# Ipsedo/MARLClassification

Measured on AMD Instinct MI355X. Metric: agent-env-steps/sec, higher is better.
Workload: dtype f32; 1 GPU; RESISC45 256x256x3, 16 agents, 16 steps, f=12, README dims (configs[2]); full train iteration: rollout + A2C loss + BPTT backward + Adam; batch_per_gpu=256, global_batch=256, parallelism=dp1, rng=library (Philox4x32-10), launch=eager

## Files before the change

marlclassification_amd/csrc/episode.hip:

```cpp
#include <math.h>
#include <stdlib.h>
#include <string.h>

#include "../../include/marl_hip_rowops.h"
#include "../../include/marl_hip_cnnops.h"
#include "../../include/marl_hip_explore.h"
#include "../../include/marl_hip_classloss.h"
#include "../../include/marl_hip_softtargets.h"
#include "common.h"

namespace marl {

struct Dims {
    int na, nb, ns;
    int64_t R, NR;
    int H, W, c_img, f;
    int L;
    int ch[MARL_MAX_CNN_LAYERS + 1];
    int grp[MARL_MAX_CNN_LAYERS];
    int hw[MARL_MAX_CNN_LAYERS + 1];
    int P[MARL_MAX_CNN_LAYERS];
    int K[MARL_MAX_CNN_LAYERS];
    int ldk[MARL_MAX_CNN_LAYERS];
    int nf, nin;
// ... 1503 lines not shown
                    MARL_P_PRE_LNW, MARL_P_PRE_LNB, NR, d.nlb, grads, 0));
    MARL_TRY(tn(c, c.at(c.e.DAQ1), d.ld_nlb, c.Hs(1), d.ld_nb, MARL_P_PRE_W0, d.nlb, d.n_b, NR, grads[MARL_P_PRE_B0]));
    MARL_TRY(tn(c, c.at(c.e.DVAL), 4, c.at(c.e.AC1), d.ld_nla, MARL_P_CRI_W1, 1, d.nla, NR, grads[MARL_P_CRI_B1]));
    if (d.nla <= 384) {
        MARL_TRY(ln_bwd_rank(c, c.at(c.e.DVAL), 4, 1, MARL_P_CRI_W1, c.at(c.e.ZC1), d.ld_nla,
                             c.at(c.e.STC1), MARL_P_CRI_LNW, MARL_P_CRI_LNB, NR, d.nla, grads,
                             c.at(c.e.DAC1), d.ld_nla));
    } else {
        MARL_TRY(gemm1(c, gemm_prob(c.at(c.e.DVAL), 4, c.wtB(MARL_P_CRI_W1), c.at(c.e.DAC1),
                                    d.ld_nla, (int)NR, d.nla)));
        MARL_TRY(ln_bwd(c, c.at(c.e.DAC1), d.ld_nla, c.at(c.e.ZC1), d.ld_nla, c.at(c.e.STC1),
                        MARL_P_CRI_LNW, MARL_P_CRI_LNB, NR, d.nla, grads, 0));
    }
    MARL_TRY(tn(c, c.at(c.e.DAC1), d.ld_nla, c.HCs(1), d.ld_na, MARL_P_CRI_W0, d.nla, d.n_a, NR, grads[MARL_P_CRI_B0]));
    if (sb && sb->g_probs) g_probs = sb->g_probs;
    const Explore& ex = c.opt.explore;
    if (ex.on && (ex.inv_tau != 1.f || ex.eps != 0.f))
        MARL_TRY(launch_policy_dlogits_explore(g_logp, g_probs, c.PROBSs(0), c.ACTs(0), c.at(c.e.DLOG), d.ld_nA, NR,
                                               d.nA, ex.inv_tau, ex.keep, ex.eps / (float)d.nA, st));
    else if (g_probs)
        MARL_TRY(launch_policy_dlogits_probs(g_logp, g_probs, c.PROBSs(0), c.ACTs(0), c.at(c.e.DLOG),
                                             d.ld_nA, NR, d.nA, st));
    else
        MARL_TRY(launch_policy_dlogits(g_logp, c.PROBSs(0), c.ACTs(0), c.at(c.e.DLOG), d.ld_nA, NR,
                                       d.nA, st));
    MARL_TRY(tn(c, c.at(c.e.DLOG), d.ld_nA, c.at(c.e.AP1, 0), d.ld_nla, MARL_P_POL_W1, d.nA, d.nla, NR, grads[MARL_P_POL_B1]));
    if (d.nA <= 4 && d.nla <= 384) {
        MARL_TRY(ln_bwd_rank(c, c.at(c.e.DLOG), d.ld_nA, d.nA, MARL_P_POL_W1, c.at(c.e.ZP1, 0),
                             d.ld_nla, c.at(c.e.STP1, 0), MARL_P_POL_LNW, MARL_P_POL_LNB, NR, d.nla,
                             grads, c.at(c.e.DAP1), d.ld_nla));
    } else {
        MARL_TRY(gemm1(c, gemm_prob(c.at(c.e.DLOG), d.ld_nA, c.wtB(MARL_P_POL_W1),
                                    c.at(c.e.DAP1), d.ld_nla, (int)NR, d.nla)));
        MARL_TRY(ln_bwd(c, c.at(c.e.DAP1), d.ld_nla, c.at(c.e.ZP1, 0), d.ld_nla, c.at(c.e.STP1, 0),
                        MARL_P_POL_LNW, MARL_P_POL_LNB, NR, d.nla, grads, 0));
    }
    MARL_TRY(tn(c, c.at(c.e.DAP1), d.ld_nla, c.HCs(1), d.ld_na, MARL_P_POL_W0, d.nla, d.n_a, NR, grads[MARL_P_POL_B0]));
    {
        GemmProb ph = gemm_prob(c.at(c.e.DAQ1), d.ld_nlb, c.wtB(MARL_P_PRE_W0), c.DHs(1), d.ld_nb, (int)NR, d.n_b);
        GemmProb pa = gemm_prob(c.at(c.e.DAP1), d.ld_nla, c.wtB(MARL_P_POL_W0), c.DHCs(1), d.ld_na, (int)NR, d.n_a);
        gemm_add_seg(pa, c.at(c.e.DAC1), d.ld_nla, c.wtB(MARL_P_CRI_W0));
        MARL_TRY(gemm2(c, ph, pa));
    }
    if (sb) {
        MARL_TRY(launch_acc2d(c.DHs(ns), d.ld_nb, sb->g_h, d.n_b, d.R, d.n_b, st));
        MARL_TRY(launch_acc2d(c.DHCs(ns), d.ld_na, sb->g_hc, d.n_a, d.R, d.n_a, st));
    }

    s.heads_early = c.opt.heads_event != nullptr && !sb;
    if (s.heads_early) {
        if (c.tq) MARL_TRY(launch_tn_queue(s.tq, c.rq, st));
        MARL_TRY(s.rq.flush());
        MARL_TRY(unpack_grads(c, grads, 1));
        MARL_HIP_CHECK(hipEventRecord(c.opt.heads_event, st));
    }
    return MARL_OK;
}


static int enc_bwd_rows(const BwdState& s, int t, int acc, float* dh) {
    const Ctx& c = s.c;
    const Dims& d = c.d;
    const int R = (int)d.R;
    float* dze2 = c.at(c.e.DZE2) + (size_t)t * d.R * d.ld_nm;
    float* dae1 = c.at(c.e.DAE1) + (size_t)t * d.R * d.ld_nm2;
    MARL_TRY(ln_bwd(c, dze2, d.ld_nm, c.at(c.e.ZE2, t), d.ld_nm, c.at(c.e.STE2, t), MARL_P_ENC_LN1W,
                    MARL_P_ENC_LN1B, d.R, d.n_m, s.grads, acc));
    MARL_TRY(gemm1(c, gemm_prob(dze2, d.ld_nm, c.wtB(MARL_P_ENC_W1), dae1, d.ld_nm2, R, d.nm2)));
    MARL_TRY(ln_bwd(c, dae1, d.ld_nm2, c.at(c.e.ZE1, t), d.ld_nm2, c.at(c.e.STE1, t), MARL_P_ENC_LN0W,
                    MARL_P_ENC_LN0B, d.R, d.nm2, s.grads, acc));
    return gemm1(c, gemm_prob(dae1, d.ld_nm2, c.wtB(MARL_P_ENC_W0), dh, d.ld_nb, R, d.n_b, nullptr, 1));
}

static int bwd_recurrent(const BwdState& s, int t, float* ddbar, float* ddbar2) {
    const Ctx& c = s.c;
    const Dims& d = c.d;
    const int R = (int)d.R;
    const struct { int which, w, row0; float* out; int ldo, n, acc; } prod[4] = {
        {0, MARL_P_LB_WHH, 0, c.DHs(t), d.ld_nb, d.n_b, 1},
        {1, MARL_P_LA_WHH, 0, c.DHCs(t), d.ld_na, d.n_a, 1},
        {0, MARL_P_LB_WIH, d.nf, ddbar, d.ld_dbl, d.n_mo + d.n_d, 0},
        {1, MARL_P_LA_WIH, d.nf, ddbar2, d.ld_dbl, d.n_mo + d.n_d, 0}};
    const int count = c.plan.panels_bwd ? 4 : 2;
    if (c.plan.panels_bwd && c.e.g3) {
        G3Batch g{};
        for (int i = 0; i < count; ++i) {
            const auto& q = prod[i];
            g.p[i] = g3_prob(c.img(q.which ? c.e.GA3 : c.e.GB3), (int)((int64_t)t * d.R), c.wt3k(q.w), q.row0,
                             4 * (q.which ? d.n_a : d.n_b), q.out, q.ldo, R, q.n, nullptr, q.acc);
        }
        g.count = count;
        return launch_gemm_nt3(g, c.st);
    }
    GemmBatch gb{};
    for (int i = 0; i < count; ++i) {
        const auto& q = prod[i];
        gb.p[i] = gemm_prob(c.at(q.which ? c.e.GA : c.e.GB, t), q.which ? d.ld_ga : d.ld_gb,
                            c.wtB(q.w).from_row(q.row0), q.out, q.ldo, R, q.n, nullptr, q.acc);
    }
    gb.count = count;
    if (!c.plan.panels_bwd) {
        GemmProb& p = gb.p[gb.count++];
        p = gemm_prob(c.at(c.e.GB, t), d.ld_gb, c.wtB(MARL_P_LB_WIH).from_row(d.nf), ddbar, d.ld_dbl, R, d.n_mo);
        gemm_add_seg(p, c.at(c.e.GA, t), d.ld_ga, c.wtB(MARL_P_LA_WIH).from_row(d.nf));
    }
    return launch_gemm_nt(gb, c.st);
}

static void fill_dec_bwd_prob(BwdState& s, int t, float* ddbar, float* ddbar2, PanelBwdProb& pd) {
    const Ctx& c = s.c;
    const Dims& d = c.d;
    pd.da = ddbar;
    pd.ldda = d.ld_dbl;
    pd.da2 = ddbar2;
    pd.ldda2 = d.ld_dbl;
    pd.m = (int)d.R;
    pd.nlayers = 2;
    fill_dec_bwd_layers(c, t, (size_t)s.pln_blocks * 2, ddbar, c.at(c.e.DAD1) + (size_t)t * d.R * d.ld_nm2, pd.layer);
    pd.dx = c.at(c.e.DMBAR);
    pd.lddx = d.ld_nm;
    pd.accumulate = 0;
    if (t > 0) {
        pd.has_cell = 1;
        pd.cell = cell_bwd_args(c, 1, t - 1);
        pd.cell_rows = d.R;
        s.action_done = true;
    }
}

static int bwd_step_chain(BwdState& s, int t, float* ddbar, float* ddbar2) {
    const Ctx& c = s.c;
    const Dims& d = c.d;
    PanelBwdProb pd{};
    fill_dec_bwd_prob(s, t, ddbar, ddbar2, pd);
    pd.by_batch = panel_chain_by_batch(d.na);
    pd.g_na = d.na;
    pd.g_nb = d.nb;
    if (t > 0) {
        pd.nlayers = 4;
        pd.agg_at = 2;
        pd.mix = c.opt.comm;
        if (c.opt.comm) pd.gate = comm_gate(c, t);
        fill_enc_bwd_layers(c, t - 1, (size_t)s.pln_blocks * 2, pd.layer + 2);
        pd.dx = c.DHs(t);
        pd.lddx = d.ld_nb;
        pd.accumulate = 1;
        pd.has_cellb = 1;
        pd.cellb = cell_bwd_args(c, 0, t - 1);
        s.belief_done = true;
    }
    MARL_TRY(launch_panel_bwd(pd, c.st));
    return gate_image_fallback(c, pd, t - 1);
}

static int bwd_step_panels(BwdState& s, int t, float* ddbar, float* ddbar2) {
    const Ctx& c = s.c;
    const Dims& d = c.d;
    PanelBwdProb pd{};
    fill_dec_bwd_prob(s, t, ddbar, ddbar2, pd);
    MARL_TRY(launch_panel_bwd(pd, c.st));
    MARL_TRY(gate_image_fallback(c, pd, t - 1));
    if (t == 0) return MARL_OK;
    PanelBwdProb pe{};
    pe.da = c.at(c.e.DMBAR);
    pe.ldda = d.ld_nm;
    pe.agg_na = d.na;
    pe.agg_nb = d.nb;
    if (c.opt.comm) {
        MARL_TRY(mix_msg(c, t, c.at(c.e.DMBAR), c.at(c.e.DMBAR), d.ld_nm, 1));
        pe.agg_na = pe.agg_nb = 0;
    }
    pe.m = (int)d.R;
    pe.nlayers = 2;
    fill_enc_bwd_layers(c, t - 1, (size_t)s.pln_blocks * 2, pe.layer);
    pe.dx = c.DHs(t);
    pe.lddx = d.ld_nb;
    pe.accumulate = 1;
    return launch_panel_bwd(pe, c.st);
}

static int bwd_step_rows(const BwdState& s, int t, float* ddbar) {
    const Ctx& c = s.c;
    const Dims& d = c.d;
// ... 1472 lines not shown
```

marlclassification_amd/csrc/panel.hip:

```cpp
#include <stdlib.h>

#include "common.h"
#include "sample.h"

namespace marl {

typedef float f32x4 __attribute__((ext_vector_type(4)));

__device__ __forceinline__ void lds_barrier() {
    asm volatile("s_waitcnt lgkmcnt(0)\n\ts_barrier" ::: "memory");
}
__device__ __forceinline__ float mul_rn(float a, float b) {
#pragma clang fp contract(off)
    return a * b;
}
__device__ __forceinline__ float silu_p(float y) { return silu_fast(y); }
__device__ __forceinline__ float silu_grad_p(float y) { return silu_grad_fast(y); }

constexpr int kPanelRows = 16;
constexpr int kPanelMaxWaves = 12;
constexpr int kPanelMaxCols = 6;

__host__ __device__ inline int panel_stride(int k) { return ((k + 15) & ~15) + 4; }

// ... 66 lines not shown
    return ks < 1 ? 1 : ks;
}

constexpr int panel_kper_c(int K16, int ks) { return (((K16 + ks - 1) / ks) + 15) & ~15; }
constexpr int panel_ksplit_c(int K, int nt, int nwaves) {
    const int K16 = (K + 15) & ~15, want = (K16 + 63) / 64;
    int ks = nwaves / nt;
    ks = ks < want ? ks : want;
    return ks < 1 ? 1 : ks;
}
constexpr int panel_stride_c(int k) { return ((k + 15) & ~15) + 4; }
constexpr int cmax(int a, int b) { return a > b ? a : b; }

struct PanelDyn {
    static constexpr bool kStatic = false, kByBatch = false;
    static constexpr int kLayers = kPanelMaxLayers, kSoft = 0, kWaves = 0, kK0 = 0, kAggAt = 0, kKLast = 0;
    static constexpr int off_e = 0, off_prm = 0, off_colp = 0, off_part = 0, off_rowmap = 0;
    static constexpr int n(int) { return 0; }
    static constexpr int k(int) { return 0; }
};
template <int WAVES, int K0, int AGG_AT, int SOFT, int... N>
struct PanelNet {
    static constexpr bool kStatic = true, kByBatch = AGG_AT > 0;
    static constexpr int kLayers = (int)sizeof...(N), kSoft = SOFT, kWaves = WAVES, kK0 = K0, kAggAt = AGG_AT;
    static constexpr int n(int l) {
        constexpr int w[] = {N...};
        return w[l];
    }
    static constexpr int k(int l) { return l == 0 ? K0 : n(l - 1); }
    static constexpr int s0(int layers) {
        int v = kPanelRows * panel_stride_c(K0);
        for (int l = 1; l < layers; l += 2) v = cmax(v, kPanelRows * panel_stride_c(n(l)));
        return v;
    }
    static constexpr int s1(int layers) {
        int v = 0;
        for (int l = 0; l < layers; l += 2) v = cmax(v, kPanelRows * panel_stride_c(n(l)));
        return v;
    }
    static constexpr bool ok() {
        for (int l = 0; l < kLayers; ++l) {
            const int nt = (n(l) + 31) >> 5, K16 = (k(l) + 15) & ~15, ks = panel_ksplit_c(k(l), nt, WAVES);
            if (nt * ks > WAVES || (ks - 1) * panel_kper_c(K16, ks) >= K16) return false;
            if ((n(l) & 15) || (k(l) & 15) || n(l) > 64 * kPanelMaxCols) return false;
        }
        return WAVES >= 4 && WAVES <= kPanelMaxWaves && (SOFT == 0 || (s0(SOFT) == s0(kLayers) && s1(SOFT) == s1(kLayers)));
    }
};
template <int WAVES, int AGG_AT, int KLAST, int... N>
struct PanelBwdNet {
    static constexpr bool kStatic = true, kByBatch = true;
    static constexpr int kLayers = (int)sizeof...(N), kSoft = 0, kWaves = WAVES, kAggAt = AGG_AT, kKLast = KLAST;
    static constexpr int n(int l) {
        constexpr int w[] = {N...};
        return w[l];
    }
    static constexpr int k(int l) { return l + 1 < kLayers ? n(l + 1) : KLAST; }
    static constexpr int nmax() {
        int v = 0;
        for (int l = 0; l < kLayers; ++l) v = cmax(v, n(l));
        return v;
    }
    static constexpr int pmax() {
        int v = 0;
        for (int l = 0; l < kLayers; ++l) v = cmax(v, cmax(panel_stride_c(n(l)), panel_stride_c(k(l))));
        return v;
    }
    static constexpr int prm() {
        int v = 0;
        for (int l = 0; l < kLayers; ++l) v += 2 * n(l);
        return v;
    }
    static constexpr int off_e = kPanelRows * pmax(), off_prm = 2 * kPanelRows * pmax(), off_colp = off_prm + prm() + 16;
    static constexpr int off_part = off_colp + WAVES * 2 * nmax(), off_rowmap = off_part + (WAVES - 1) * 512;
    static constexpr bool ok() {
        for (int l = 0; l < kLayers; ++l) {
            const int nt = (k(l) + 31) >> 5, n16 = (n(l) + 15) & ~15, ks = panel_ksplit_c(n(l), nt, WAVES);
            if (nt > WAVES || (ks - 1) * panel_kper_c(n16, ks) >= n16) return false;
            if ((n(l) & 15) || (k(l) & 15)) return false;
        }
        return WAVES >= 8 && WAVES <= kPanelMaxWaves && nmax() <= 128 && (KLAST & 3) == 0;
    }
};

template <int K16, int KS, int KPER>
__device__ __forceinline__ void panel_gemm_st(f32x4 (&acc)[2], const float* in, int stride,
                                              const float* __restrict__ wfrag, int j, int s, int lane) {
    constexpr int groups = K16 >> 4, last0 = (KS - 1) * KPER;
    static_assert(last0 < K16 && (KPER & 15) == 0, "slice plan");
    const int quad = lane >> 4, l16 = lane & 15;
    const int kbeg = __builtin_amdgcn_readfirstlane(s * KPER);
    const float* arow = in + l16 * stride + 4 * quad + kbeg;
    const int g0 = __builtin_amdgcn_readfirstlane(j * groups + (kbeg >> 4));
    const float* wb = wfrag + (size_t)g0 * 512;
    const unsigned lo = 4u * (unsigned)lane;
#pragma unroll
    for (int r = 0; r < 4; ++r) acc[0][r] = acc[1][r] = 0.f;
#pragma unroll
    for (int c = 0; c < (KPER + 63) / 64; ++c) {
        if (last0 + 64 * c < K16 || kbeg + 64 * c < K16) {
            float4 b0[4], b1[4];
#pragma unroll
            for (int i = 0; i < 4; ++i) {
                if (64 * c + 16 * i < KPER) {
                    b0[i] = *reinterpret_cast<const float4*>(wb + 2048 * c + 512 * i + lo);
                    b1[i] = *reinterpret_cast<const float4*>(wb + 2048 * c + 512 * i + 256 + lo);
                }
            }
#pragma unroll
            for (int i = 0; i < 4; ++i) {
                if (64 * c + 16 * i < KPER && (last0 + 64 * c + 16 * i < K16 || kbeg + 64 * c + 16 * i < K16)) {
                    const float4 a = *reinterpret_cast<const float4*>(arow + 64 * c + 16 * i);
                    acc[0] = __builtin_amdgcn_mfma_f32_16x16x4f32(a.x, b0[i].x, acc[0], 0, 0, 0);
                    acc[1] = __builtin_amdgcn_mfma_f32_16x16x4f32(a.x, b1[i].x, acc[1], 0, 0, 0);
                    acc[0] = __builtin_amdgcn_mfma_f32_16x16x4f32(a.y, b0[i].y, acc[0], 0, 0, 0);
                    acc[1] = __builtin_amdgcn_mfma_f32_16x16x4f32(a.y, b1[i].y, acc[1], 0, 0, 0);
                    acc[0] = __builtin_amdgcn_mfma_f32_16x16x4f32(a.z, b0[i].z, acc[0], 0, 0, 0);
                    acc[1] = __builtin_amdgcn_mfma_f32_16x16x4f32(a.z, b1[i].z, acc[1], 0, 0, 0);
                    acc[0] = __builtin_amdgcn_mfma_f32_16x16x4f32(a.w, b0[i].w, acc[0], 0, 0, 0);
                    acc[1] = __builtin_amdgcn_mfma_f32_16x16x4f32(a.w, b1[i].w, acc[1], 0, 0, 0);
                }
            }
        }
    }
}

template <class SH, bool BWD, int L = 0>
__device__ __forceinline__ void panel_gemm_layer(int l, f32x4 (&acc)[2], const float* in, int stride,
                                                 const float* __restrict__ wfrag, int j, int s, int lane) {
    if constexpr (SH::kStatic && L < SH::kLayers) {
        if (l == L) {
            constexpr int K = BWD ? SH::n(L) : SH::k(L), nout = BWD ? SH::k(L) : SH::n(L);
            constexpr int K16 = (K + 15) & ~15, ks = panel_ksplit_c(K, (nout + 31) >> 5, SH::kWaves);
            panel_gemm_st<K16, ks, panel_kper_c(K16, ks)>(acc, in, stride, wfrag, j, s, lane);
        } else {
            panel_gemm_layer<SH, BWD, L + 1>(l, acc, in, stride, wfrag, j, s, lane);
        }
    }
}

template <int NC>
__device__ __forceinline__ void panel_ln_rows(const PanelLayer& Lr, float* outp, int ys, int n, const float* lgamma,
                                              const float* lbeta, const int* rowmap, int wave, int nwaves, int lane)
{
    constexpr int RPW = 4;
    float g[NC], bt[NC];
#pragma unroll
    for (int u = 0; u < NC; ++u) {
        const int c = lane + 64 * u;
        g[u] = c < n ? lgamma[c] : 0.f;
        bt[u] = c < n ? lbeta[c] : 0.f;
    }
    const float inv_n = 1.0f / (float)n;
#pragma unroll
    for (int i = 0; i < RPW; ++i) {
        const int lr = wave + i * nwaves;
        if (lr < kPanelRows) {
            float* zr = outp + lr * ys;
            const int row = rowmap[lr];
            float v[NC];
            float sm = 0.f;
#pragma unroll
            for (int u = 0; u < NC; ++u) {
                const int c = lane + 64 * u;
                v[u] = c < n ? zr[c] : 0.f;
                sm += v[u];
// ... 726 lines not shown
    {
        float pv[kPanelMaxLayers][2];
#pragma unroll
        for (int l = 0; l < kPanelMaxLayers; ++l) {
            pv[l][0] = pv[l][1] = 0.f;
            if (ST && l >= SH::kLayers) continue;
            if (l < nlayers && tid < (ST ? SH::n(l) : P.layer[l].n)) {
                pv[l][0] = P.layer[l].gamma[tid];
                pv[l][1] = P.layer[l].beta[tid];
            }
        }
        float cmv = 0.f;
        if (MIX && !GATE && tid < P.g_na * P.g_na) {
            const int a = tid / P.g_na, a2 = tid - a * P.g_na;
            cmv = P.mix[a2 * P.g_na + a];
        }
        if (MIX && GATE && tid < bpb * P.g_na * P.g_na) {
            const int na = P.g_na, i = tid / (na * na), e = tid - i * na * na, a = e / na;
            const int b = (int)blockIdx.x * bpb + i;
            if (b < P.g_nb) cmv = comm_gate_weight<kPanelRows>(P.mix, P.gate, na, P.g_nb, b, e - a * na, a);
        }
        int off = 0;
#pragma unroll
        for (int l = 0; l < kPanelMaxLayers; ++l) {
            if (ST && l >= SH::kLayers) continue;
            if (l < nlayers) {
                const int n = ST ? SH::n(l) : P.layer[l].n;
                if (tid < n) {
                    prm[off + tid] = pv[l][0];
                    prm[off + n + tid] = pv[l][1];
                }
                off += 2 * n;
            }
        }
        if (MIX && !GATE && tid < P.g_na * P.g_na) lds[P.off_mix + tid] = cmv;
        if (MIX && GATE && tid < bpb * P.g_na * P.g_na) lds[P.off_mix + tid] = cmv;
        const int n = ST ? SH::n(0) : P.layer[0].n, ds = panel_stride(n), n16 = (n + 15) & ~15, c4 = n16 >> 2;
        const int n4 = (n + 3) & ~3;
        const int agg_na = ST ? 0 : P.agg_na;
        for (int e = tid; e < kPanelRows * c4; e += nthreads) {
            const int lr = e / c4, k = (e % c4) * 4;
            const int r = rowmap[lr];
            float4 v = make_float4(0.f, 0.f, 0.f, 0.f);
            if (r >= 0 && k < n4 && agg_na > 1) {
                const int na = P.agg_na, nb = P.agg_nb;
                const float den = (float)(na - 1);
                const float* base = P.da + (size_t)(r % nb) * P.ldda + k;
                const size_t astr = (size_t)nb * P.ldda;
                float4 s = make_float4(0.f, 0.f, 0.f, 0.f);
                for (int a0 = 0; a0 < na; a0 += 8) {
                    float4 qv[8];
#pragma unroll
                    for (int u = 0; u < 8; ++u) {
                        const int a = a0 + u < na ? a0 + u : na - 1;
                        qv[u] = *reinterpret_cast<const float4*>(base + (size_t)a * astr);
                    }
#pragma unroll
                    for (int u = 0; u < 8; ++u) {
                        if (a0 + u < na) {
                            s.x += qv[u].x;
                            s.y += qv[u].y;
                            s.z += qv[u].z;
                            s.w += qv[u].w;
                        }
                    }
                }
                const float4 me = *reinterpret_cast<const float4*>(P.da + (size_t)r * P.ldda + k);
                v = make_float4((s.x - me.x) / den, (s.y - me.y) / den, (s.z - me.z) / den,
                                (s.w - me.w) / den);
            } else if (r >= 0 && k < n4 && agg_na == 0) {
                v = *reinterpret_cast<const float4*>(P.da + (size_t)r * P.ldda + k);
                if (P.da2) {
                    const float4 w = *reinterpret_cast<const float4*>(P.da2 + (size_t)r * P.ldda2 + k);
                    v = make_float4(v.x + w.x, v.y + w.y, v.z + w.z, v.w + w.w);
                }
            }
            *reinterpret_cast<float4*>(D + lr * ds + k) = v;
        }
    }
    MARL_TS();
    lds_barrier();
    MARL_TS();

    int prm_off = 0;
    constexpr int kUnroll = ST ? SH::kLayers : 1;
#pragma unroll kUnroll
    for (int l = 0; l < nlayers; ++l) {
        const PanelBwdLayer Lr = P.layer[l];
        const int n = ST ? SH::n(l) : Lr.n, ds = panel_stride(n), n16 = (n + 15) & ~15;
        const float* lgamma = prm + prm_off;
        const float* lbeta = lgamma + n;
        prm_off += 2 * n;
        if (l > 0 && l == (ST ? SH::kAggAt : P.agg_at)) {
            const int c4 = n16 >> 2, na = P.g_na;
            const float den = (float)(na - 1);
            float4 v[2];
#pragma unroll
            for (int it = 0; it < 2; ++it) {
                const int e = tid + it * nthreads;
                v[it] = make_float4(0.f, 0.f, 0.f, 0.f);
                if (e < kPanelRows * c4) {
                    const int lr = e / c4, k = (e - lr * c4) * 4;
                    const int a = lr / bpb, i = lr - a * bpb;
                    if (MIX) {
                        if (a < na) {
                            const float* crow = lds + P.off_mix + (GATE ? i * na + a : a) * na;
                            float4 sm = make_float4(0.f, 0.f, 0.f, 0.f);
                            for (int a2 = 0; a2 < na; ++a2) {
                                const float cf = crow[a2];
                                if (cf != 0.f) {
                                    const float4 q = *reinterpret_cast<const float4*>(D + (a2 * bpb + i) * ds + k);
                                    sm.x = fmaf(cf, q.x, sm.x);
                                    sm.y = fmaf(cf, q.y, sm.y);
                                    sm.z = fmaf(cf, q.z, sm.z);
                                    sm.w = fmaf(cf, q.w, sm.w);
                                }
                            }
                            v[it] = sm;
                        }
                    } else if (a < na && na > 1) {
                        float4 sm = make_float4(0.f, 0.f, 0.f, 0.f);
                        for (int a2 = 0; a2 < na; ++a2) {
                            const float4 q = *reinterpret_cast<const float4*>(D + (a2 * bpb + i) * ds + k);
                            sm.x += q.x;
                            sm.y += q.y;
                            sm.z += q.z;
                            sm.w += q.w;
                        }
                        const float4 me = *reinterpret_cast<const float4*>(D + lr * ds + k);
                        v[it] = make_float4((sm.x - me.x) / den, (sm.y - me.y) / den, (sm.z - me.z) / den,
                                            (sm.w - me.w) / den);
                    }
                }
            }
            lds_barrier();
#pragma unroll
            for (int it = 0; it < 2; ++it) {
                const int e = tid + it * nthreads;
                if (e < kPanelRows * c4) {
                    const int lr = e / c4, k = (e - lr * c4) * 4;
                    *reinterpret_cast<float4*>(D + lr * ds + k) = v[it];
                }
            }
            lds_barrier();
        }
        {
            constexpr int RPW = 2;
            float pg[MAXC], pb[MAXC], g[MAXC], bt[MAXC];
#pragma unroll
            for (int u = 0; u < MAXC; ++u) {
                const int c = lane + 64 * u;
                pg[u] = pb[u] = 0.f;
                g[u] = c < n ? lgamma[c] : 0.f;
                bt[u] = c < n ? lbeta[c] : 0.f;
            }
            const float inv_n = 1.0f / (float)n;
#pragma unroll
            for (int i = 0; i < RPW; ++i) {
                const int lr = wave + i * nwaves;
                if (lr < kPanelRows) {
                    const int row = rowmap[lr];
                    const bool rv = row >= 0;
                    float xh[MAXC], dxh[MAXC];
                    float s1 = 0.f, s2 = 0.f, rstd = 0.f;
                    if (rv) {
                        const float mean = mpre[i];
                        rstd = rpre[i];
#pragma unroll
                        for (int u = 0; u < MAXC; ++u) {
                            const int c = lane + 64 * u;
                            xh[u] = dxh[u] = 0.f;
                            if (c < n) {
                                xh[u] = (zpre[i][u] - mean) * rstd;
                                const float dy = mul_rn(D[lr * ds + c], silu_grad_p(g[u] * xh[u] + bt[u]));
                                dxh[u] = mul_rn(dy, g[u]);
                                s1 += dxh[u];
                                s2 += mul_rn(dxh[u], xh[u]);
                                pg[u] += mul_rn(dy, xh[u]);
                                pb[u] += dy;
                            }
                        }
                    } else {
#pragma unroll
                        for (int u = 0; u < MAXC; ++u) xh[u] = dxh[u] = 0.f;
                    }
                    const float m1 = wave_sum(s1) * inv_n, m2 = wave_sum(s2) * inv_n;
#pragma unroll
                    for (int u = 0; u < MAXC; ++u) {
                        const int c = lane + 64 * u;
                        if (c < n16) {
                            float dzv = 0.f;
                            if (rv && c < n) {
                                dzv = rstd * (dxh[u] - m1 - xh[u] * m2);
                                Lr.dz[(size_t)row * Lr.lddz + c] = dzv;
                            }
                            D[lr * ds + c] = dzv;
                        }
                    }
                }
            }
            float* cw = colp + (size_t)wave * 2 * n;
#pragma unroll
            for (int u = 0; u < MAXC; ++u) {
                const int c = lane + 64 * u;
                if (c < n) {
                    cw[c] = pg[u];
                    cw[n + c] = pb[u];
                }
            }
        }
        MARL_TS();
        lds_barrier();
        MARL_TS();
        for (int c = tid; c < 2 * n; c += nthreads) {
            float t = 0.f;
            for (int w = 0; w < nwaves; ++w) t += colp[(size_t)w * 2 * n + c];
            Lr.part[(size_t)blockIdx.x * 2 * n + c] = t;
        }
        if (l + 1 < nlayers) zfetch(P.layer[l + 1], ST ? SH::n(l + 1 < SH::kLayers ? l + 1 : 0) : P.layer[l + 1].n);
        MARL_TS();
        const int nout = ST ? SH::k(l) : Lr.k_in, nt = (nout + 31) >> 5;
        const int ks = panel_ksplit(n, nt, nwaves);
        const int kper = (((n16 + ks - 1) / ks) + 15) & ~15;
        const bool last = l + 1 == nlayers;
        const bool tail_lds = ST || P.tail_lds;
        const int es = panel_stride(nout), o16 = (nout + 15) & ~15;
        for (int t0 = 0; t0 < nt; t0 += nwaves / ks) {
            const int tiles_round = nwaves / ks;
            const int j = t0 + wave % tiles_round, s = wave / tiles_round;
            const bool active = s < ks && j < nt;
            f32x4 acc[2];
            if constexpr (ST) {
                if (active) panel_gemm_layer<SH, true>(l, acc, D, ds, Lr.wtfrag, j, s, lane);
            } else {
                const int kbeg = s * kper;
                const int kend = kbeg + kper < n16 ? kbeg + kper : n16;
                if (active) panel_gemm(acc, D, ds, Lr.wtfrag, Lr.wgroups, j, kbeg, kend, lane);
            }
            panel_ksum(acc, part, tiles_round, ks, wave % tiles_round, s, lane, active);
            if (active && s == 0) {
                int rw[4];
#pragma unroll
                for (int r = 0; r < 4; ++r) rw[r] = last ? rowmap[4 * quad + r] : -1;
#pragma unroll
                for (int t = 0; t < 2; ++t) {
                    const int col = j * 32 + 16 * t + l16;
#pragma unroll
                    for (int r = 0; r < 4; ++r) {
                        const int lr = 4 * quad + r;
                        const int row = rw[r];
                        const float v = col < nout ? acc[t][r] : 0.f;
                        if (last && tail_lds) {
                            if (col < o16) E[lr * es + col] = v;
                        } else if (last) {
                            if (col < nout && row >= 0) {
                                float* o = P.dx + (size_t)row * P.lddx + col;
                                const float tot = P.accumulate ? *o + v : v;
                                *o = tot;
                                if (P.has_cellb) lstm_cell_bwd_at(P.cellb, row, col, tot);
                            }
                        } else if (col < o16) {
                            E[lr * es + col] = v;
                        }
                    }
                }
            }
            lds_barrier();
        }
        MARL_TS();
        if (last && tail_lds) {
            const LstmBwdArgs& Cb = P.cellb;
            const int c4n = nout >> 2, items = kPanelRows * c4n, cn = ST ? nout : Cb.n;
            constexpr int kIt = 1;
            for (int base = 0; base < items; base += kIt * nthreads) {
                float4 ov[kIt], gi[kIt], gf[kIt], gg[kIt], go[kIt], cnew[kIt], cprev[kIt], dcv[kIt];
                int rowi[kIt], coli[kIt], lri[kIt];
#pragma unroll
                for (int k = 0; k < kIt; ++k) {
                    const int i = base + tid + k * nthreads;
                    const int lr = i < items ? i / c4n : 0;
                    const int c = i < items ? (i - lr * c4n) * 4 : 0;
                    const int row = i < items ? rowmap[lr] : -1;
                    const size_t rr = row < 0 ? 0 : (size_t)row;
                    rowi[k] = row;
                    coli[k] = c;
                    lri[k] = lr;
                    ov[k] = P.accumulate ? *reinterpret_cast<const float4*>(P.dx + rr * P.lddx + c)
                                         : make_float4(0.f, 0.f, 0.f, 0.f);
                    if (P.has_cellb) {
                        const float* g = Cb.gates + rr * Cb.ldg + c;
                        gi[k] = *reinterpret_cast<const float4*>(g);
                        gf[k] = *reinterpret_cast<const float4*>(g + cn);
                        gg[k] = *reinterpret_cast<const float4*>(g + 2 * cn);
                        go[k] = *reinterpret_cast<const float4*>(g + 3 * cn);
                        cnew[k] = *reinterpret_cast<const float4*>(Cb.c_new + rr * Cb.ldc + c);
                        cprev[k] = *reinterpret_cast<const float4*>(Cb.c_prev + rr * Cb.ldc + c);
                        dcv[k] = *reinterpret_cast<const float4*>(Cb.dc + rr * Cb.lddc + c);
                    }
                }
#pragma unroll
                for (int k = 0; k < kIt; ++k) {
                    if (rowi[k] < 0) continue;
                    const float4 v = *reinterpret_cast<const float4*>(E + lri[k] * es + coli[k]);
                    const float tot[4] = {ov[k].x + v.x, ov[k].y + v.y, ov[k].z + v.z, ov[k].w + v.w};
                    *reinterpret_cast<float4*>(P.dx + (size_t)rowi[k] * P.lddx + coli[k]) =
                        make_float4(tot[0], tot[1], tot[2], tot[3]);
                    if (P.has_cellb) {
                        const float gi_[4] = {gi[k].x, gi[k].y, gi[k].z, gi[k].w};
                        const float gf_[4] = {gf[k].x, gf[k].y, gf[k].z, gf[k].w};
                        const float gg_[4] = {gg[k].x, gg[k].y, gg[k].z, gg[k].w};
                        const float go_[4] = {go[k].x, go[k].y, go[k].z, go[k].w};
                        const float cn_[4] = {cnew[k].x, cnew[k].y, cnew[k].z, cnew[k].w};
                        const float cp_[4] = {cprev[k].x, cprev[k].y, cprev[k].z, cprev[k].w};
                        const float dc_[4] = {dcv[k].x, dcv[k].y, dcv[k].z, dcv[k].w};
                        float o0[4], o1[4], o2[4], o3[4], o4[4];
#pragma unroll
                        for (int q = 0; q < 4; ++q) {
                            const float tc = tanh_fast(cn_[q]);
                            const float d = tot[q] * go_[q] * (1.0f - tc * tc) + dc_[q];
                            o0[q] = d * gg_[q] * gi_[q] * (1.0f - gi_[q]);
                            o1[q] = d * cp_[q] * gf_[q] * (1.0f - gf_[q]);
                            o2[q] = d * gi_[q] * (1.0f - gg_[q] * gg_[q]);
                            o3[q] = tot[q] * tc * go_[q] * (1.0f - go_[q]);
                            o4[q] = d * gf_[q];
                        }
                        if (!(Cb.g3 && Cb.skip_f32)) {
                            float* g = Cb.gates + (size_t)rowi[k] * Cb.ldg + coli[k];
                            *reinterpret_cast<float4*>(g) = make_float4(o0[0], o0[1], o0[2], o0[3]);
                            *reinterpret_cast<float4*>(g + cn) = make_float4(o1[0], o1[1], o1[2], o1[3]);
                            *reinterpret_cast<float4*>(g + 2 * cn) = make_float4(o2[0], o2[1], o2[2], o2[3]);
                            *reinterpret_cast<float4*>(g + 3 * cn) = make_float4(o3[0], o3[1], o3[2], o3[3]);
                        }
                        *reinterpret_cast<float4*>(Cb.dc + (size_t)rowi[k] * Cb.lddc + coli[k]) =
                            make_float4(o4[0], o4[1], o4[2], o4[3]);
                        if (Cb.g3) {
                            const int64_t ir = (int64_t)Cb.g3_row0 + rowi[k];
                            const int c0 = coli[k];
                            img_store4(Cb.g3 + img_off(ir, c0 >> 4, Cb.g3_steps), c0, o0[0], o0[1], o0[2], o0[3]);
                            img_store4(Cb.g3 + img_off(ir, (cn + c0) >> 4, Cb.g3_steps), cn + c0, o1[0], o1[1], o1[2], o1[3]);
                            img_store4(Cb.g3 + img_off(ir, (2 * cn + c0) >> 4, Cb.g3_steps), 2 * cn + c0, o2[0], o2[1], o2[2], o2[3]);
                            img_store4(Cb.g3 + img_off(ir, (3 * cn + c0) >> 4, Cb.g3_steps), 3 * cn + c0, o3[0], o3[1], o3[2], o3[3]);
                        }
                    }
                }
            }
        }
        MARL_TS();
        float* tmp = D;
        D = E;
        E = tmp;
    }
}

int panel_bwd_blocks(int m) { return (int)cdiv(m, kPanelRows); }
int panel_chain_blocks(int na, int nb) { return na >= 1 && na <= kPanelRows ? (int)cdiv(nb, kPanelRows / na) : 0; }
int panel_chain_by_batch(int na) { return na >= 1 && na <= kPanelRows ? kPanelRows / na : 0; }

struct PanelBwdPlan {
    int waves, maxc;
    size_t lds;
    unsigned pblocks, cblocks;
    bool retried;
};
static int panel_bwd_plan(PanelBwdProb& p, PanelBwdPlan& pl) {
    int waves = 8, pmax = 0, nmax = 0, prm = 0;
    pl.retried = false;
    const PanelBwdLayer& Ll = p.layer[p.nlayers - 1];
    bool tail_lds = (Ll.k_in & 3) == 0 && (p.lddx & 3) == 0 &&
                    (!p.has_cellb || ((p.cellb.n & 3) == 0 && (p.cellb.ldg & 3) == 0 && (p.cellb.ldc & 3) == 0 &&
                                      (p.cellb.lddc & 3) == 0 && p.cellb.n == Ll.k_in)) &&
                    true;
plan:
    waves = 8;
    pmax = nmax = prm = 0;
    p.tail_lds = tail_lds ? 1 : 0;
    for (int l = 0; l < p.nlayers; ++l) {
        const PanelBwdLayer& L = p.layer[l];
        if (!L.wtfrag) {
            set_error("panel backward: layer %d has no fragment-order copy of its transposed weight", l);
            return MARL_EINVAL;
        }
        if (L.wgroups != panel_frag_groups(L.n)) {
            set_error("panel backward: layer %d's weight copy has %d groups, its width %d needs %d", l, L.wgroups, L.n,
                      panel_frag_groups(L.n));
            return MARL_ELIMIT;
        }
        if (L.n > 64 * kBwdMaxCols) {
            set_error("panel backward: LayerNorm width %d > %d", L.n, 64 * kBwdMaxCols);
            return MARL_ELIMIT;
        }
        int w = panel_waves_for(L.n, L.k_in);
        if (w < 0) w = kPanelMaxWaves;
        waves = w > waves ? w : waves;
        nmax = L.n > nmax ? L.n : nmax;
        pmax = panel_stride(L.n) > pmax ? panel_stride(L.n) : pmax;
        if ((l + 1 < p.nlayers || tail_lds) && panel_stride(L.k_in) > pmax) pmax = panel_stride(L.k_in);
        prm += 2 * L.n;
// ... 521 lines not shown
```

Before: 9.615 million agent-env-steps/s.

## Skip recurrent-state grads at step zero and prefetch LSTM tail operands early

At the first timestep of backward, the recurrent hidden-state gradient GEMMs (W_hh products) are dropped and only the input/message gradient products are launched, reusing the original kernel variant. Their outputs feed nothing earlier in time. In the static panel-backward kernel, the LSTM cell backward operands (gates, c states, dc, dx) are loaded into registers before the last layer's LN/GEMM work rather than after it, hiding global load latency. The risks are higher register pressure from the prefetch and a possible correctness issue if those step-zero gradients were consumed elsewhere.

Result: no change. 9.705 million agent-env-steps/s, median of 6 (+0.9%).

```diff
diff --git a/marlclassification_amd/csrc/episode.hip b/marlclassification_amd/csrc/episode.hip
--- a/marlclassification_amd/csrc/episode.hip
+++ b/marlclassification_amd/csrc/episode.hip
@@ -1609,6 +1609,7 @@
         {0, MARL_P_LB_WIH, d.nf, ddbar, d.ld_dbl, d.n_mo + d.n_d, 0},
         {1, MARL_P_LA_WIH, d.nf, ddbar2, d.ld_dbl, d.n_mo + d.n_d, 0}};
     const int count = c.plan.panels_bwd ? 4 : 2;
+    const bool msg_only = c.plan.panels_bwd && !s.sb && t == 0;
     if (c.plan.panels_bwd && c.e.g3) {
         G3Batch g{};
         for (int i = 0; i < count; ++i) {
@@ -1617,6 +1618,13 @@
                              4 * (q.which ? d.n_a : d.n_b), q.out, q.ldo, R, q.n, nullptr, q.acc);
         }
         g.count = count;
+        if (msg_only) {
+            const int variant = g3_nt_plan(g).variant;
+            g.p[0] = g.p[2];
+            g.p[1] = g.p[3];
+            g.count = 2;
+            return launch_gemm_nt3(g, c.st, variant);
+        }
         return launch_gemm_nt3(g, c.st);
     }
     GemmBatch gb{};
@@ -1626,6 +1634,15 @@
                             c.wtB(q.w).from_row(q.row0), q.out, q.ldo, R, q.n, nullptr, q.acc);
     }
     gb.count = count;
+    if (msg_only) {
+        GemmBatch g2 = gb;
+        g2.p[0] = gb.p[2];
+        g2.p[1] = gb.p[3];
+        g2.count = 2;
+        const GemmPlan pl4 = gemm_nt_plan(gb), pl2 = gemm_nt_plan(g2);
+        if (pl4.family == pl2.family && pl4.bm == pl2.bm && pl4.bn == pl2.bn && pl4.single_buf == pl2.single_buf)
+            return launch_gemm_nt(g2, c.st);
+    }
     if (!c.plan.panels_bwd) {
         GemmProb& p = gb.p[gb.count++];
         p = gemm_prob(c.at(c.e.GB, t), d.ld_gb, c.wtB(MARL_P_LB_WIH).from_row(d.nf), ddbar, d.ld_dbl, R, d.n_mo);
diff --git a/marlclassification_amd/csrc/panel.hip b/marlclassification_amd/csrc/panel.hip
--- a/marlclassification_amd/csrc/panel.hip
+++ b/marlclassification_amd/csrc/panel.hip
@@ -172,6 +172,19 @@
         return WAVES >= 8 && WAVES <= kPanelMaxWaves && nmax() <= 128 && (KLAST & 3) == 0;
     }
 };
+
+template <int N>
+struct PanelTailOps {
+    float4 ov[N], gi[N], gf[N], gg[N], go[N], cnew[N], cprev[N], dcv[N];
+};
+template <class SH>
+constexpr int panel_tail_items() {
+    if constexpr (SH::kStatic) {
+        return (kPanelRows * (SH::kKLast >> 2) + 64 * SH::kWaves - 1) / (64 * SH::kWaves);
+    } else {
+        return 1;
+    }
+}
 
 template <int K16, int KS, int KPER>
 __device__ __forceinline__ void panel_gemm_st(f32x4 (&acc)[2], const float* in, int stride,
@@ -1064,6 +1077,57 @@
     lds_barrier();
     MARL_TS();
 
+    constexpr int kIt = panel_tail_items<SH>();
+    auto tail_item = [&](const int i, const int c4n, int& lr, int& c, int& row) {
+        const int items = kPanelRows * c4n;
+        lr = i < items ? i / c4n : 0;
+        c = i < items ? (i - lr * c4n) * 4 : 0;
+        row = i < items ? rowmap[lr] : -1;
+    };
+    auto tail_fetch = [&](PanelTailOps<kIt>& o, const int base, const int c4n, const int cn) {
+        const LstmBwdArgs& Cb = P.cellb;
+        const bool hc = P.has_cellb != 0;
+        const float *bg = hc ? Cb.gates : P.dx, *bn = hc ? Cb.c_new : P.dx, *bp = hc ? Cb.c_prev : P.dx;
+        const float* bd = hc ? Cb.dc : P.dx;
+        const int sg = hc ? Cb.ldg : P.lddx, sc = hc ? Cb.ldc : P.lddx, sd = hc ? Cb.lddc : P.lddx, gs = hc ? cn : 0;
+        if constexpr (ST) asm volatile("" : "+s"(bg), "+s"(bn), "+s"(bp), "+s"(bd));
+#pragma unroll
+        for (int k = 0; k < kIt; ++k) {
+            int lr, c, row;
+            tail_item(base + tid + k * nthreads, c4n, lr, c, row);
+            const size_t rr = row < 0 ? 0 : (size_t)row;
+            if constexpr (ST) {
+                auto gp4 = [](const float* p) {
+                    const f32x4 v = *(const __attribute__((address_space(1))) f32x4*)p;
+                    return make_float4(v[0], v[1], v[2], v[3]);
+                };
+                const float* g = bg + rr * sg + c;
+                o.ov[k] = gp4(P.dx + rr * P.lddx + c);
+                o.gi[k] = gp4(g);
+                o.gf[k] = gp4(g + gs);
+                o.gg[k] = gp4(g + 2 * gs);
+                o.go[k] = gp4(g + 3 * gs);
+                o.cnew[k] = gp4(bn + rr * sc + c);
+                o.cprev[k] = gp4(bp + rr * sc + c);
+                o.dcv[k] = gp4(bd + rr * sd + c);
+                continue;
+            }
+            o.ov[k] = P.accumulate ? *reinterpret_cast<const float4*>(P.dx + rr * P.lddx + c)
+                                   : make_float4(0.f, 0.f, 0.f, 0.f);
+            if (P.has_cellb) {
+                const float* g = Cb.gates + rr * Cb.ldg + c;
+                o.gi[k] = *reinterpret_cast<const float4*>(g);
+                o.gf[k] = *reinterpret_cast<const float4*>(g + cn);
+                o.gg[k] = *reinterpret_cast<const float4*>(g + 2 * cn);
+                o.go[k] = *reinterpret_cast<const float4*>(g + 3 * cn);
+                o.cnew[k] = *reinterpret_cast<const float4*>(Cb.c_new + rr * Cb.ldc + c);
+                o.cprev[k] = *reinterpret_cast<const float4*>(Cb.c_prev + rr * Cb.ldc + c);
+                o.dcv[k] = *reinterpret_cast<const float4*>(Cb.dc + rr * Cb.lddc + c);
+            }
+        }
+    };
+    PanelTailOps<kIt> pre;
+
     int prm_off = 0;
     constexpr int kUnroll = ST ? SH::kLayers : 1;
 #pragma unroll kUnroll
@@ -1126,6 +1190,9 @@
             }
             lds_barrier();
         }
+        if constexpr (ST) {
+            if (l + 1 == nlayers) tail_fetch(pre, 0, SH::kKLast >> 2, SH::kKLast);
+        }
         {
             constexpr int RPW = 2;
             float pg[MAXC], pb[MAXC], g[MAXC], bt[MAXC];
@@ -1253,48 +1320,29 @@
         if (last && tail_lds) {
             const LstmBwdArgs& Cb = P.cellb;
             const int c4n = nout >> 2, items = kPanelRows * c4n, cn = ST ? nout : Cb.n;
-            constexpr int kIt = 1;
             for (int base = 0; base < items; base += kIt * nthreads) {
-                float4 ov[kIt], gi[kIt], gf[kIt], gg[kIt], go[kIt], cnew[kIt], cprev[kIt], dcv[kIt];
+                PanelTailOps<kIt> o;
+                if constexpr (ST) o = pre;
+                else tail_fetch(o, base, c4n, cn);
                 int rowi[kIt], coli[kIt], lri[kIt];
 #pragma unroll
-                for (int k = 0; k < kIt; ++k) {
-                    const int i = base + tid + k * nthreads;
-                    const int lr = i < items ? i / c4n : 0;
-                    const int c = i < items ? (i - lr * c4n) * 4 : 0;
-                    const int row = i < items ? rowmap[lr] : -1;
-                    const size_t rr = row < 0 ? 0 : (size_t)row;
-                    rowi[k] = row;
-                    coli[k] = c;
-                    lri[k] = lr;
-                    ov[k] = P.accumulate ? *reinterpret_cast<const float4*>(P.dx + rr * P.lddx + c)
-                                         : make_float4(0.f, 0.f, 0.f, 0.f);
-                    if (P.has_cellb) {
-                        const float* g = Cb.gates + rr * Cb.ldg + c;
-                        gi[k] = *reinterpret_cast<const float4*>(g);
-                        gf[k] = *reinterpret_cast<const float4*>(g + cn);
-                        gg[k] = *reinterpret_cast<const float4*>(g + 2 * cn);
-                        go[k] = *reinterpret_cast<const float4*>(g + 3 * cn);
-                        cnew[k] = *reinterpret_cast<const float4*>(Cb.c_new + rr * Cb.ldc + c);
-                        cprev[k] = *reinterpret_cast<const float4*>(Cb.c_prev + rr * Cb.ldc + c);
-                        dcv[k] = *reinterpret_cast<const float4*>(Cb.dc + rr * Cb.lddc + c);
-                    }
-                }
+                for (int k = 0; k < kIt; ++k) tail_item(base + tid + k * nthreads, c4n, lri[k], coli[k], rowi[k]);
 #pragma unroll
                 for (int k = 0; k < kIt; ++k) {
                     if (rowi[k] < 0) continue;
                     const float4 v = *reinterpret_cast<const float4*>(E + lri[k] * es + coli[k]);
-                    const float tot[4] = {ov[k].x + v.x, ov[k].y + v.y, ov[k].z + v.z, ov[k].w + v.w};
+                    if (ST && !P.accumulate) o.ov[k] = make_float4(0.f, 0.f, 0.f, 0.f);
+                    const float tot[4] = {o.ov[k].x + v.x, o.ov[k].y + v.y, o.ov[k].z + v.z, o.ov[k].w + v.w};
                     *reinterpret_cast<float4*>(P.dx + (size_t)rowi[k] * P.lddx + coli[k]) =
                         make_float4(tot[0], tot[1], tot[2], tot[3]);
                     if (P.has_cellb) {
-                        const float gi_[4] = {gi[k].x, gi[k].y, gi[k].z, gi[k].w};
-                        const float gf_[4] = {gf[k].x, gf[k].y, gf[k].z, gf[k].w};
-                        const float gg_[4] = {gg[k].x, gg[k].y, gg[k].z, gg[k].w};
-                        const float go_[4] = {go[k].x, go[k].y, go[k].z, go[k].w};
-                        const float cn_[4] = {cnew[k].x, cnew[k].y, cnew[k].z, cnew[k].w};
-                        const float cp_[4] = {cprev[k].x, cprev[k].y, cprev[k].z, cprev[k].w};
-                        const float dc_[4] = {dcv[k].x, dcv[k].y, dcv[k].z, dcv[k].w};
+                        const float gi_[4] = {o.gi[k].x, o.gi[k].y, o.gi[k].z, o.gi[k].w};
+                        const float gf_[4] = {o.gf[k].x, o.gf[k].y, o.gf[k].z, o.gf[k].w};
+                        const float gg_[4] = {o.gg[k].x, o.gg[k].y, o.gg[k].z, o.gg[k].w};
+                        const float go_[4] = {o.go[k].x, o.go[k].y, o.go[k].z, o.go[k].w};
+                        const float cn_[4] = {o.cnew[k].x, o.cnew[k].y, o.cnew[k].z, o.cnew[k].w};
+                        const float cp_[4] = {o.cprev[k].x, o.cprev[k].y, o.cprev[k].z, o.cprev[k].w};
+                        const float dc_[4] = {o.dcv[k].x, o.dcv[k].y, o.dcv[k].z, o.dcv[k].w};
                         float o0[4], o1[4], o2[4], o3[4], o4[4];
 #pragma unroll
                         for (int q = 0; q < 4; ++q) {
```
